# p-m-mueller/saddle_point_petsc

Measured on AMD Instinct MI355X. Metric: FGMRES iterations/sec + achieved HBM GB/s on A-block SpMV, 1/2/4/8 MI355X, higher is better.
Workload: dtype f64

## Files before the change

### include/spk.h

```cpp
#ifndef SPK_H
#define SPK_H

#include <stdint.h>

#ifdef __cplusplus
extern "C" {
#endif

#define SPK_VERSION 100

typedef struct spk_ctx spk_ctx;

enum { SPK_OK = 0, SPK_ERR_ARG = -1, SPK_ERR_HIP = -2, SPK_ERR_STATE = -3,
       SPK_ERR_COMM = -4, SPK_ERR_NOMEM = -5, SPK_ERR_UNSUPPORTED = -6 };

enum { SPK_MEM_HOST = 0, SPK_MEM_DEVICE = 1 };

enum { SPK_BLOCK_A00 = 0, SPK_BLOCK_A10 = 1 };

enum { SPK_PC_NONE = 0, SPK_PC_JACOBI = 1, SPK_PC_SCHUR = 2 };
enum { SPK_SCHUR_DIAG = 0, SPK_SCHUR_LOWER = 1, SPK_SCHUR_UPPER = 2, SPK_SCHUR_FULL = 3 };
enum { SPK_ORTHOG_CGS = 0, SPK_ORTHOG_MGS = 1 };
enum { SPK_REFINE_NEVER = 0, SPK_REFINE_IFNEEDED = 1, SPK_REFINE_ALWAYS = 2 };
enum { SPK_SPMV_CSR = 0 };
// ... 181 lines not shown
int spk_kernel_mdot(spk_ctx *ctx, int64_t n, int32_t nv, const double *V, int64_t ldv,
                    const double *w, double *h);
int spk_kernel_maxpy(spk_ctx *ctx, int64_t n, int32_t nv, const double *a, const double *V,
                     int64_t ldv, double *w, double *nrm2);
int spk_time_spmv(spk_ctx *ctx, int warmup, int reps, double *ms_per_launch);
int spk_time_kernel(spk_ctx *ctx, const char *which, int nv, int warmup, int reps,
                    double *ms_per_launch);

int spk_debug_finish_timeout(spk_ctx *ctx, int timeout_ms);

int spk_debug_wave_sums(spk_ctx *ctx, int na, const double *in, double *out);

#define SPK_DEBUG_MARKER (-7777777.0)
int spk_debug_vec_shape(spk_ctx *ctx, int64_t n, int32_t *out);
typedef struct spk_debug_mdot_opts {
    int64_t n, n_dot;
    int32_t nv, nv2;
    int32_t split, done;
    double pad;
} spk_debug_mdot_opts;
int spk_debug_mdot(spk_ctx *ctx, const spk_debug_mdot_opts *o, const double *V, const double *V2, const double *w, double *out);
typedef struct spk_debug_maxpy_opts {
    int64_t n, n_dot, n_bd;
    double sign, pad;
    int32_t nv, nv_live;
    int32_t want_norm;
    int32_t m, bd_mode;
    int32_t w1side, pyth, done;
} spk_debug_maxpy_opts;
int spk_debug_maxpy(spk_ctx *ctx, const spk_debug_maxpy_opts *o, const double *V, const double *a, double *w, const double *bd,
                    const double *dots, double *tb, double *red, double *w1side, double *nrm_out);
int spk_debug_cycle_norm(spk_ctx *ctx, int64_t n, int64_t n_dot, int64_t n_bd, int32_t m, double pad, double *x, const double *sa,
                         const double *sb, const double *bd, double *red, double *w1side);
int spk_debug_schur_w(spk_ctx *ctx, int64_t nl, int32_t m, int32_t fact, int32_t done, double pad, const double *W, const double *L,
                      const double *x, const double *src, const double *dinv, double *y);
int spk_debug_pack_bd(spk_ctx *ctx, int64_t n, int32_t m, const double *bd, double *bdp, int32_t *bad);
typedef struct spk_debug_head_opts {
    int64_t nl;
    int32_t m, packed, fact, jacobi, want_wl, reserved;
    double pad;
} spk_debug_head_opts;
int spk_debug_cycle_head(spk_ctx *ctx, const spk_debug_head_opts *o, double *v, const double *nrm, const double *w1raw,
                         const double *dinv, const double *bd, const double *shat, const double *gram, double *z, double *c,
                         double *wl);

int spk_debug_gs_stamps(spk_ctx *ctx, uint64_t *out);

int spk_debug_set_wait_bound(spk_ctx *ctx, uint32_t ticks);

int spk_debug_time_products(spk_ctx *ctx, int32_t max_launches);
int spk_get_product_timing(spk_ctx *ctx, int32_t *launches, double *mean_ms, double *median_ms, double *min_ms, double *max_ms,
                           int32_t *gated, double *gated_mean_ms);

int spk_partition_slab(int64_t nlines, int64_t line_rows, int rank, int nranks,
                       int64_t *row_begin, int64_t *row_end);
int spk_partition_split(int64_t row_begin, int32_t nrows_local, const int32_t *rowptr,
                        const int32_t *colidx, const double *val,
                        int32_t *d_rowptr, int32_t *d_colidx, double *d_val,
                        int32_t *o_rowptr, int32_t *o_colidx, double *o_val,
                        int32_t *garray, int64_t *nnz_d, int64_t *nnz_o, int32_t *n_ghost);

#ifdef __cplusplus
}
#endif
#endif
```

### saddle_point_petsc_amd/_lib.py

```python
import ctypes as C
import os

import numpy as np

_HERE = os.path.dirname(os.path.abspath(__file__))
LIB_PATH = os.path.join(_HERE, "libspk.so")

i32p = np.ctypeslib.ndpointer(np.int32, flags="C_CONTIGUOUS")
f64p = np.ctypeslib.ndpointer(np.float64, flags="C_CONTIGUOUS")


class SpkError(RuntimeError):
    def __init__(self, code, msg):
        super().__init__(f"libspk error {code}: {msg}")
        self.code = code


class Opts(C.Structure):
    _fields_ = [
        ("restart", C.c_int32), ("max_it", C.c_int32), ("rtol", C.c_double),
        ("abstol", C.c_double), ("dtol", C.c_double), ("guess_nonzero", C.c_int32),
        ("orthog", C.c_int32), ("check_every", C.c_int32), ("fused", C.c_int32),
        ("cgs_refine", C.c_int32), ("single_reduce", C.c_int32), ("iteration_form", C.c_int32), ("reserved", C.c_int32),
    ]
# ... 107 lines not shown
    _hip_preloaded = _preload_hip_runtime()
    L = C.CDLL(LIB_PATH)
    rts = hip_runtimes_mapped()
    if len(rts) > 1:
        raise ImportError("two HIP runtimes are mapped into this process (" + ", ".join(rts) + "): libspk.so would not find the "
                          "GPU.  Import saddle_point_petsc_amd before anything else that loads a HIP runtime of its own, or set "
                          "LD_LIBRARY_PATH so that both resolve libamdhip64.so.7 to the same file.")
    vp, i32, i64, dbl = C.c_void_p, C.c_int32, C.c_int64, C.c_double
    L.spk_version.restype = C.c_int
    L.spk_last_error.restype = C.c_char_p
    L.spk_last_error.argtypes = [vp]
    L.spk_default_opts.argtypes = [C.POINTER(Opts)]
    L.spk_default_opts.restype = None
    L.spk_create.argtypes = [C.POINTER(vp), C.c_int]
    L.spk_destroy.argtypes = [vp]
    L.spk_comm_unique_id.argtypes = [C.c_char_p]
    L.spk_comm_init_rccl.argtypes = [vp, C.c_int, C.c_int, C.c_char_p]
    L.spk_comm_init_host.argtypes = [vp, C.c_int, C.c_int, C.POINTER(HostComm)]
    L.spk_local_group_create.argtypes = [C.POINTER(vp), C.c_int]
    L.spk_local_group_destroy.argtypes = [vp]
    L.spk_comm_init_local.argtypes = [vp, vp, C.c_int]
    L.spk_comm_enable_peer.argtypes = [vp, C.POINTER(i32)]
    L.spk_comm_backend.restype = C.c_char_p
    L.spk_comm_backend.argtypes = [vp]
    L.spk_comm_get_info.argtypes = [vp, C.POINTER(CommInfo)]
    L.spk_debug_peer_allreduce_loopback.argtypes = [vp, C.c_int, C.c_int, C.c_int, f64p, f64p]
    L.spk_debug_finish_timeout.argtypes = [vp, C.c_int]
    L.spk_debug_set_wait_bound.argtypes = [vp, C.c_uint32]
    L.spk_debug_wave_sums.argtypes = [vp, C.c_int, f64p, f64p]
    L.spk_debug_vec_shape.argtypes = [vp, i64, i32p]
    L.spk_debug_mdot.argtypes = [vp, C.POINTER(DebugMdotOpts), vp, vp, f64p, f64p]
    L.spk_debug_maxpy.argtypes = [vp, C.POINTER(DebugMaxpyOpts), vp, f64p, f64p, vp, vp, vp, f64p, vp, vp]
    L.spk_debug_cycle_norm.argtypes = [vp, i64, i64, i64, i32, dbl, f64p, vp, vp, vp, f64p, vp]
    L.spk_debug_schur_w.argtypes = [vp, i64, i32, i32, i32, dbl, f64p, f64p, f64p, vp, vp, f64p]
    L.spk_debug_pack_bd.argtypes = [vp, i64, i32, f64p, vp, C.POINTER(i32)]
    L.spk_debug_cycle_head.argtypes = [vp, C.POINTER(DebugHeadOpts), f64p, f64p, vp, f64p, vp, vp, vp, f64p, vp, vp]
    L.spk_debug_gs_stamps.argtypes = [vp, np.ctypeslib.ndpointer(np.uint64, flags="C_CONTIGUOUS")]
    L.spk_debug_time_products.argtypes = [vp, C.c_int32]
    L.spk_get_product_timing.argtypes = [vp, C.POINTER(C.c_int32)] + [C.POINTER(C.c_double)] * 4 + [C.POINTER(C.c_int32), C.POINTER(C.c_double)]
    L.spk_set_block.argtypes = [vp, C.c_int, i64, i32, i64, i32p, i32p, f64p]
    L.spk_set_block_laplace.argtypes = [vp, C.c_int, C.c_int, vp, C.c_int, C.c_int, vp]
    L.spk_assemble_laplace_csr.argtypes = [vp, C.c_int, C.c_int, i64, i64, vp, C.c_int, C.c_int, i32p, i32p, f64p, vp]
    L.spk_set_block_laplace3d.argtypes = [vp, C.c_int, C.c_int, C.c_int, vp, C.c_int, C.c_int, vp]
    L.spk_assemble_laplace3d_csr.argtypes = [vp, C.c_int, C.c_int, C.c_int, i64, i64, vp, C.c_int, C.c_int, i32p, i32p, f64p, vp]
    L.spk_get_assembly_seconds.argtypes = [vp, C.POINTER(dbl)]
    L.spk_pc_setup.argtypes = [vp, C.c_int, C.c_int]
    L.spk_pc_set_inner.argtypes = [vp, C.c_int, C.c_double]
    L.spk_default_amg_opts.argtypes = [C.POINTER(AmgOpts)]
    L.spk_default_amg_opts.restype = None
    L.spk_pc_set_amg.argtypes = [vp, C.POINTER(AmgOpts)]
    L.spk_get_amg_info.argtypes = [vp, C.POINTER(AmgInfo)]
    L.spk_get_amg_level.argtypes = [vp, C.c_int, C.c_int, C.POINTER(i32), C.POINTER(i32), C.POINTER(i64), vp, vp, vp]
    L.spk_get_amg_aggregates.argtypes = [vp, C.c_int, C.POINTER(i32), vp]
    L.spk_amg_build_host.argtypes = [i32, i32p, i32p, f64p, C.POINTER(AmgOpts), C.POINTER(vp)]
    L.spk_amg_refresh_host.argtypes = [vp, vp]
    L.spk_amg_destroy_host.argtypes = [vp]
    L.spk_pc_set_amg_reuse.argtypes = [vp, C.c_int]
    L.spk_get_amg_reuse_info.argtypes = [vp, C.POINTER(i32), C.POINTER(dbl)]
    L.spk_amg_host_info.argtypes = [vp, C.POINTER(AmgInfo)]
    L.spk_amg_host_level.argtypes = [vp, C.c_int, C.c_int, C.POINTER(i32), C.POINTER(i32), C.POINTER(i64), vp, vp, vp]
    L.spk_amg_host_aggregates.argtypes = [vp, C.c_int, C.POINTER(i32), vp]
    L.spk_pc_set_schur_pre.argtypes = [vp, C.c_int]
    L.spk_get_schur_matrix.argtypes = [vp, f64p]
    L.spk_get_schur_setup_seconds.argtypes = [vp, C.POINTER(dbl)]
    L.spk_get_schur_diag.argtypes = [vp, f64p]
    L.spk_get_jacobi_diag.argtypes = [vp, f64p]
# ... 81 lines not shown
```

### saddle_point_petsc_amd/csrc/spk_api.cpp

```cpp
#include <algorithm>
#include <cmath>
#include <cstdlib>
#include <cstring>
#include <string>

#include "spk_internal.hpp"

namespace spk {
void rccl_unique_id(void *id128);
}

static thread_local std::string g_create_error;
namespace spk {
void set_create_error(const std::string &m) { g_create_error = m; }
}

#define SPK_TRY(ctx)                                                     \
    if (!(ctx)) return SPK_ERR_ARG;                                      \
    try {                                                                \
        if (hipSetDevice((ctx)->device) != hipSuccess)                   \
            spk::fail(SPK_ERR_HIP, "hipSetDevice(%d) failed", (ctx)->device);

#define SPK_CATCH(ctx)                                                   \
    }                                                                    \
// ... 670 lines not shown
    spk::DevBuf<double> dV, dw, da, dbd, ddots, dtb, dred, dside, dnrm;
    spk::DevBuf<int32_t> ddone, dnv;
    dbg_upload(dV, V, o->nv, n, ld, o->pad);
    dbg_upload(dw, w, 1, n, ld, o->pad);
    dbg_upload(dbd, bd, rows, n, ld, o->pad);
    da.upload(a, (size_t)o->nv, 8);
    dbg_fill(dred, (size_t)(1 + m), SPK_DEBUG_MARKER);
    dbg_fill(dside, (size_t)std::max(m, 1), SPK_DEBUG_MARKER);
    dbg_fill(dnrm, (size_t)(1 + m), SPK_DEBUG_MARKER);
    spk::k::PythArgs py{};
    py.m = -1;
    if (o->pyth) {
        ddots.upload(dots, (size_t)(live + m + 1), 8);
        dtb.upload(tb, (size_t)(o->nv + 1) * 8, 8);
        py = spk::k::PythArgs{m, ddots.p, dtb.p, dnrm.p};
    }
    if (o->nv_live >= 0) dnv.upload(&o->nv_live, 1, 3);
    const int32_t *done = dbg_done(ddone, o->done);
    spk::k::maxpy(dV.p, ld, o->nv, o->nv_live >= 0 ? dnv.p : nullptr, da.p, o->sign, dw.p, n, o->n_dot,
                  c->fin(o->want_norm ? dred.p : nullptr), done, c->stream, rows ? dbd.p : nullptr, ld, o->n_bd, m,
                  o->w1side ? dside.p : nullptr, o->pyth ? &py : nullptr, o->bd_mode == 2);
    SPK_HIP(hipStreamSynchronize(c->stream));
    c->check_device_error();
    SPK_HIP(hipMemcpy(w, dw.p, sizeof(double) * (size_t)n, hipMemcpyDeviceToHost));
    SPK_HIP(hipMemcpy(red, dred.p, sizeof(double) * (size_t)(1 + m), hipMemcpyDeviceToHost));
    if (w1side && m) SPK_HIP(hipMemcpy(w1side, dside.p, sizeof(double) * (size_t)m, hipMemcpyDeviceToHost));
    if (o->pyth) {
        SPK_HIP(hipMemcpy(nrm_out, dnrm.p, sizeof(double) * (size_t)(1 + m), hipMemcpyDeviceToHost));
        SPK_HIP(hipMemcpy(tb, dtb.p, sizeof(double) * (size_t)(o->nv + 1) * 8, hipMemcpyDeviceToHost));
    }
    SPK_CATCH(c)
}

int spk_debug_cycle_norm(spk_ctx *c, int64_t n, int64_t n_dot, int64_t n_bd, int32_t m, double pad, double *x, const double *sa,
                         const double *sb, const double *bd, double *red, double *w1side)
{
    SPK_TRY(c)
    if (!x || !red || n <= 0 || n_dot < 0 || n_dot > n || n_bd < 0 || n_bd + m > n || m < 0 || m > 8 || (m && (!bd || !w1side)) ||
        (!sa != !sb))
        spk::fail(SPK_ERR_ARG, "spk_debug_cycle_norm: bad arguments");
    c->ensure_scratch();
    const int64_t ld = dbg_ld(n);
    spk::DevBuf<double> dx, dsa, dsb, dbd, dred, dside;
    dbg_upload(dx, sa ? nullptr : x, 1, n, ld, pad);
    if (sa) {
        dbg_upload(dsa, sa, 1, n, ld, pad);
        dbg_upload(dsb, sb, 1, n, ld, pad);
    }
    dbg_upload(dbd, bd, m, n, ld, pad);
    dbg_fill(dred, (size_t)(1 + m), SPK_DEBUG_MARKER);
    dbg_fill(dside, (size_t)std::max<int>(m, 1), SPK_DEBUG_MARKER);
    spk::k::sqnorm_bd(dx.p, n, n_dot, dbd.p, ld, n_bd, m, dside.p, c->fin(dred.p), nullptr, c->stream, sa ? dsa.p : nullptr,
                      sa ? dsb.p : nullptr);
    SPK_HIP(hipStreamSynchronize(c->stream));
    c->check_device_error();
    SPK_HIP(hipMemcpy(x, dx.p, sizeof(double) * (size_t)n, hipMemcpyDeviceToHost));
    SPK_HIP(hipMemcpy(red, dred.p, sizeof(double) * (size_t)(1 + m), hipMemcpyDeviceToHost));
    if (m) SPK_HIP(hipMemcpy(w1side, dside.p, sizeof(double) * (size_t)m, hipMemcpyDeviceToHost));
    SPK_CATCH(c)
}

int spk_debug_schur_w(spk_ctx *c, int64_t nl, int32_t m, int32_t fact, int32_t done, double pad, const double *W, const double *L,
                      const double *x, const double *src, const double *dinv, double *y)
{
    SPK_TRY(c)
    if (!W || !L || !x || !y || nl <= 0 || m < 1 || m > 8 || fact < SPK_SCHUR_DIAG || fact > SPK_SCHUR_FULL || (src && dinv))
        spk::fail(SPK_ERR_ARG, "spk_debug_schur_w: bad arguments");
    c->ensure_scratch();
    const int64_t ld = dbg_ld(nl + m);
    spk::DevBuf<double> dW, dL, dx, dsrc, ddinv, dy;
    spk::DevBuf<int32_t> ddone;
    dbg_upload(dW, W, m, nl, ld, 0.0);
    dL.upload(L, (size_t)m * m, 8);
    dbg_upload(dx, x, 1, nl + m, ld, pad);
    if (src) dbg_upload(dsrc, src, 1, nl, ld, pad);
    if (dinv) dbg_upload(ddinv, dinv, 1, nl, ld, pad);
    dbg_upload(dy, nullptr, 1, nl + m, ld, SPK_DEBUG_MARKER);
    const int32_t *gate = dbg_done(ddone, done);
    const spk::k::SchurW w{dW.p, ld, m, dL.p};
    if (fact == SPK_SCHUR_DIAG || fact == SPK_SCHUR_UPPER) spk::k::schur_w_y1(w, fact, dx.p + nl, dy.p + nl, gate, c->stream);
    else spk::k::schur_w_dot(w, dx.p, nl, dx.p + nl, dy.p + nl, c->fin(nullptr), gate, c->stream);
    if (fact == SPK_SCHUR_UPPER || fact == SPK_SCHUR_FULL)
        spk::k::schur_w_out(w, src ? dsrc.p : dx.p, dinv ? ddinv.p : nullptr, dy.p + nl, dy.p, nl, gate, c->stream);
    SPK_HIP(hipStreamSynchronize(c->stream));
    c->check_device_error();
    SPK_HIP(hipMemcpy(y, dy.p, sizeof(double) * (size_t)ld, hipMemcpyDeviceToHost));
// ... 313 lines not shown
```

### saddle_point_petsc_amd/csrc/spk_device.hpp

```cpp
#pragma once
#include "spk_internal.hpp"
#include "spk_gs_stamps.hpp"

#include <cmath>
#include <cstdlib>
#include <type_traits>

namespace spk {
namespace k {

constexpr int kThreads = 256;
constexpr int kWave = 64;
constexpr int kVT = 1024;
constexpr int kVWaves = kVT / kWave;
constexpr int kVecUnroll = 4;
constexpr int kVecMaxBlocks = 256;

__device__ __forceinline__ double wave_sum(double v)
{
#pragma unroll
    for (int off = kWave / 2; off > 0; off >>= 1) v += __shfl_down(v, off, kWave);
    return v;
}

// ... 495 lines not shown
{
    const GivensPre pre = givens_prefetch(gr.ka, gr.loc, gr.h);
    if (gr.fin_n > 0) {
        double *red = lds;
        double *slot = gr.fin_partials + (size_t)gr.fin_n * kPartialLd;
        double lam2 = 0.0;
        if (threadIdx.x == 0) lam2 = peek(slot);
        final_reduce<2>(gr.fin_partials, gr.fin_n, kPartialLd, 1, red, gr.fe);
        if (threadIdx.x == 0) {
            publish(slot, __longlong_as_double((long long)kSentinelBits));
            red[0] = red[0] + lam2;
        }
        __syncthreads();
        if (gr.ar.P) peer_allreduce_block(gr.ar, red, 1, gr.nrm2);
        else if (threadIdx.x == 0) gr.nrm2[0] = red[0];
        __syncthreads();
    }
    if (gr.sc && threadIdx.x == 0) gr.sc[gr.loc + 1] = inv_norm(*gr.nrm2);
    givens_block_lds<true>(gr.ka, gr.loc, gr.h, gr.nrm2, lds + kThreads, kMaxNv + 2, &pre);
}

void givens_rider_alone(const GivensRider &gr, const int32_t *done, hipStream_t s);
inline GivensRider no_rider()
{
    GivensRider g{};
    g.loc = -1;
    return g;
}

struct RowTail {
    const int32_t *bt_rowptr, *bt_colidx;
    const double *bt_val, *lam;
    OffDiag od;
};

template <bool RIDE>
__device__ __forceinline__ int product_prologue(const int32_t *done, const GivensRider &gr, double *lds)
{
    if (done && *done) return -1;
    if (RIDE && blockIdx.x == 0) {
        givens_rider(gr, lds);
        return -1;
    }
    return (int)blockIdx.x - (RIDE ? 1 : 0);
}
__device__ __forceinline__ int xcd_tile(int bx, int tiles_per_xcd) { return (bx & 7) * tiles_per_xcd + (bx >> 3); }

__device__ __forceinline__ void row_tail_bt(const RowTail &t, int k, int k1, double &s)
{
    for (; k < k1; ++k) s = __builtin_fma(t.bt_val[k], t.lam[t.bt_colidx[k]], s);
}
__device__ __forceinline__ void row_tail_add(const RowTail &t, int64_t row, double &s, bool bt)
{
    if (t.od.rowptr)
        for (int k = t.od.rowptr[row]; k < t.od.rowptr[row + 1]; ++k) s = __builtin_fma(t.od.val[k], t.od.xg[t.od.colidx[k]], s);
    if (bt) row_tail_bt(t, t.bt_rowptr[row], t.bt_rowptr[row + 1], s);
}
constexpr int kBtPre = 4;
struct BtPre {
    int k0, k1;
    double v[kBtPre], l[kBtPre];
    __device__ __forceinline__ void load(const RowTail &t, int64_t row)
    {
        k0 = t.bt_rowptr[row];
        k1 = t.bt_rowptr[row + 1];
#pragma unroll
// ... 7 lines not shown
    {
#pragma unroll
        for (int j = 0; j < kBtPre; ++j)
            if (k0 + j < k1) s = __builtin_fma(v[j], l[j], s);
        row_tail_bt(t, k0 + kBtPre, k1, s);
    }
};

__device__ __forceinline__ float sweep_update(float y, float omega, float d, float x, float s)
{
#pragma clang fp contract(off)
    return y + ((omega * d) * (x - s));
}

struct ProductLaunch {
    RowTail tail;
    GivensRider gr;
    const int32_t *done;
    int nride;
    bool acc, ride, bt;
    size_t rider_lds;
};
inline bool product_is_empty(int64_t nrows, const GivensRider *rider, const int32_t *done, hipStream_t s)
{
    if (nrows == 0 && rider) givens_rider_alone(*rider, done, s);
    return nrows == 0;
}
inline ProductLaunch make_product_launch(const CsrDev *bt, const double *lam, const OffDiag *od, const GivensRider *rider,
                                         const int32_t *done, bool accumulate)
{
    if (bt && rider) fail(SPK_ERR_ARG, "A-block product: B^T rows and a rider in one launch");
    ProductLaunch p{};
    p.tail = RowTail{bt ? bt->rowptr.p : nullptr, bt ? bt->colidx.p : nullptr, bt ? bt->val.p : nullptr, lam,
                     od ? *od : OffDiag{nullptr, nullptr, nullptr, nullptr}};
    p.gr = rider ? *rider : no_rider();
    p.done = done;
    p.nride = rider ? 1 : 0;
    p.acc = accumulate;
    p.ride = rider != nullptr;
    p.bt = bt != nullptr;
    p.rider_lds = rider ? sizeof(double) * (size_t)(kThreads + 4 * (kMaxNv + 2) + 4) : 0;
    return p;
}
template <class F>
inline void dispatch_product(bool acc, bool ride, bool bt, F &&f)
{
    using Y = std::true_type;
    using N = std::false_type;
    if (bt) acc ? f(Y{}, N{}, Y{}) : f(N{}, N{}, Y{});
    else if (acc) ride ? f(Y{}, Y{}, N{}) : f(Y{}, N{}, N{});
    else ride ? f(N{}, Y{}, N{}) : f(N{}, N{}, N{});
}

struct WsShape {
    int U, grid;
    bool on;
};
inline WsShape ws_shape(int64_t n2)
{
    WsShape v;
    static const int knob = [] { const char *e = getenv("SPK_VEC_WS"); return e ? atoi(e) : -1; }();
    v.on = n2 < (int64_t)kVecMaxBlocks * 2048 && knob != 0;
    v.U = n2 >= (int64_t)kVecMaxBlocks * 64 * 8 ? 8 : (n2 >= (int64_t)kVecMaxBlocks * 64 * 4 ? 4 : 2);
    if (knob == 2 || knob == 4 || knob == 8) v.U = knob;
    int64_t tiles = (n2 + 64 * v.U - 1) / (64 * v.U);
    if (tiles < 1) tiles = 1;
    v.grid = (int)(tiles < kVecMaxBlocks ? tiles : kVecMaxBlocks);
// ... 200 lines not shown
```

### saddle_point_petsc_amd/csrc/spk_internal.hpp

```cpp
#pragma once
#include <hip/hip_runtime.h>

#include <algorithm>
#include <chrono>
#include <cstdint>
#include <cstdio>
#include <functional>
#include <memory>
#include <string>
#include <vector>

#include <hip/hip_ext.h>

#include "spk_host.hpp"
#include "spk_amg.hpp"

namespace spk {

#define SPK_HIP(call)                                                                  \
    do {                                                                               \
        hipError_t e_ = (call);                                                        \
        if (e_ != hipSuccess)                                                          \
            ::spk::fail(SPK_ERR_HIP, "%s failed: %s (%s:%d)", #call, hipGetErrorString(e_), \
                        __FILE__, __LINE__);                                           \
// ... 227 lines not shown

struct SolverWork {
    DevBuf<double> vec;
    DevBuf<double> out, hist;
    DevBuf<unsigned char> state;
    void *pin = nullptr;
    hipEvent_t ev[2] = {nullptr, nullptr};
    void ensure(int64_t ld, int nvec, int32_t hist_cap, size_t state_bytes);
    ~SolverWork();
};

namespace k {
constexpr int kMaxNv = 64;
constexpr int kBigNv = 1024;
constexpr int kPartialLd = 64;
constexpr int kMaxBlocks = 2048;
constexpr int kBTile = 512;

void build_tiles(const int32_t *rowptr, int32_t nrows, std::vector<int32_t> &tile_row);
void arm_partials(double *p, size_t n, hipStream_t s);
struct Finish;
void finish_probe(const Finish &f, hipStream_t s);
void wave_sums_probe(int na, const double *in, double *out, hipStream_t s);
void vec_shapes_probe(int64_t n, int32_t *out);

struct Finish {
    double *partials;
    double *out;
    PeerAR ar;
    int32_t *err = nullptr;
    uint32_t fin_ticks = 400000000u;
};

struct OffDiag {
    const int32_t *rowptr, *colidx;
    const double *val, *xg;
};
struct SendRanges {
    int n;
    int32_t r0[4], len[4], off[4];
    double *buf;
    int peer;
    uint32_t seq, timeout_ms;
    unsigned long long *remote[4];
    const unsigned long long *mine;
    int32_t nrecv;
    double *xghost;
    int32_t *err;
    unsigned long long *stats;
};

struct GivensRider;
void spmv(const CsrDev &A, const double *x, double *y, const CsrDev *bt, const double *lam,
          const int32_t *done, hipStream_t s, bool accumulate = false, const OffDiag *od = nullptr,
          const GivensRider *rider = nullptr);
void spmv_bcsr(const BcsrDev &A, const double *x, double *y, const CsrDev *bt, const double *lam,
               const int32_t *done, hipStream_t s, bool accumulate = false, const OffDiag *od = nullptr,
               const GivensRider *rider = nullptr);
void build_btiles(const int32_t *browptr, int32_t nbrows, std::vector<int32_t> &tile_brow);
constexpr int kB3Tile = 256;
void spmv_bcsr3(const Bcsr3Dev &A, const double *x, double *y, const CsrDev *bt, const double *lam,
                const int32_t *done, hipStream_t s, bool accumulate = false, const OffDiag *od = nullptr,
                const GivensRider *rider = nullptr);
void build_b3tiles(const int32_t *browptr, int32_t nbrows, std::vector<int32_t> &tile_brow);
constexpr int kDictMaxPat = 1024, kDictMaxBlk = 1024, kDictSlots = 8192, kDictLdsMax = 48 * 1024;
void spmv_dict(const DictDev &A, const double *x, double *y, const CsrDev *bt, const double *lam, const int32_t *done,
// ... 41 lines not shown
               double *vbot, int32_t *fail, hipStream_t s);
void assemble_laplace(int mx, int my, int j0, int j1, const double *kappa, int apply_bc, int32_t *rowptr, int32_t *colidx, double *val,
                      double *f, hipStream_t s);
int64_t assemble_laplace_grid(int mx, int j0, int j1);
void assemble_laplace3d(int mx, int my, int mz, int k0, int k1, const double *kappa, int apply_bc, int32_t *rowptr, int32_t *colidx,
                        double *val, double *f, hipStream_t s);
int64_t assemble_laplace3d_grid(int mx, int my, int k0, int k1);
void kappa_check(const double *kappa, int64_t ne, int32_t *flag, hipStream_t s);
void wide_dot(const WideDev &B, const double *x, const Finish &f, const int32_t *done, hipStream_t s,
              const int32_t *rowmap = nullptr);
void schur_diag_rows(const CsrDev &B, const double *dinv, double *shat, hipStream_t s);
void wide_dot_jacobi(const WideDev &B, const double *x, const double *dinv, const Finish &f,
                     const int32_t *done, hipStream_t s);
void scatter_row(const int32_t *colidx, const double *val, int k0, int k1, const double *dinv,
                 double *dense, hipStream_t s);
void sum_slots(const double *slots, int nslots, int ld, int count, double *out, hipStream_t s);
void mdot(const double *V, int64_t ldv, int nv, const double *w, int64_t n, int64_t n_dot,
          const Finish &f, const int32_t *done, hipStream_t s, const double *V2 = nullptr, int nv2 = 0,
          int v2_split = 0);
struct PythArgs {
    int m;
    const double *dots;
    double *tb;
    double *nrm_out;
};
void maxpy(const double *V, int64_t ldv, int nv, const int32_t *nv_dev, const double *a,
           double coef_sign, double *w, int64_t n, int64_t n_dot, const Finish &f,
           const int32_t *done, hipStream_t s, const double *bd = nullptr, int64_t ldb = 0, int64_t n_bd = 0, int m = 0,
           double *w1side = nullptr, const PythArgs *pyth = nullptr, int bd_packed = 0);
void build_bd(const CsrDev &Bt, const double *dinv, int m, int64_t ldb, double *bd, hipStream_t s);
void pack_bd(const double *bd, int64_t ldb, int64_t n, int m, double *bdp, int32_t *bad, hipStream_t s);
void sqnorm_bd(double *x, int64_t n, int64_t n_dot, const double *bd, int64_t ldb, int64_t n_bd, int m,
               double *w1side, const Finish &f, const int32_t *done, hipStream_t s, const double *sa = nullptr,
               const double *sb = nullptr);
void scale_dev(double *x, int64_t n, const double *alpha_dev, const int32_t *done, hipStream_t s);
void axpby(double a, const double *x, double b, double *y, int64_t n, const int32_t *done, hipStream_t s);
void sqnorm(const double *x, int64_t n_dot, const Finish &f, const int32_t *done, hipStream_t s);
void sqnorm_sub(const double *sa, const double *sb, double *x, int64_t n, int64_t n_dot, const Finish &f, const int32_t *done,
                hipStream_t s);
void gather(const double *x, const int32_t *idx, int64_t n, double *out, const int32_t *done, hipStream_t s);
void peer_allreduce(const PeerAR &a, double *buf, int count, hipStream_t s);
void peer_allreduce_loopback(const PeerAR &a, double *buf, int count, hipStream_t s);
void peer_exchange(const PeerHalo &h, const double *sendbuf, double *recvbuf, hipStream_t s);
void peer_exchange_bulk(const PeerBulk &h, const double *sendbuf, double *recvbuf, hipStream_t s);
void jacobi(const double *dinv, const double *x, double *y, int64_t n, const int32_t *done, hipStream_t s);
void extract_diag_inv(const CsrDev &A, double *dinv, hipStream_t s);
void bt_update(int mode, const CsrDev &Bt, const double *dinv, const double *x0, const double *y1,
               double *y0, const int32_t *done, hipStream_t s, double *scratch = nullptr);
void cvt_scale_f32(const double *x, const float *d32, float omega, float *x32, float *y32, int64_t n,
                   const int32_t *done, hipStream_t s);
void jacobi_sweep_f32(const CsrDev &A, const float *val32, const float *d32, float omega, const float *x32,
                      const float *yin, float *yout, const int32_t *done, hipStream_t s);
void sweep_offdiag_f32(const CsrDev &Ao, const int32_t *rows, const float *d32, float omega, const double *xg,
                       float *y, const int32_t *done, hipStream_t s);
void gather_f32(const float *x, const int32_t *idx, int64_t n, double *out, const int32_t *done, hipStream_t s);
void cvt_f32_out(const float *y32, double *y, int mode, int64_t n, const int32_t *done, hipStream_t s);
void cvt_vals_f32(const double *v, float *v32, int64_t n, hipStream_t s);
void schur_y1(int fact, int m, const double *x1, const double *t, const double *shat, double *y1,
              const int32_t *done, hipStream_t s);
void copy_small(const double *src, double *dst, int n, const int32_t *done, hipStream_t s);
struct SchurW {
    const double *W;
    int64_t ldw;
    int m;
    const double *L;
};
void schur_w_dot(const SchurW &w, const double *x0, int64_t nl, const double *x1, double *y1, const Finish &f,
// ... 421 lines not shown
```

### saddle_point_petsc_amd/csrc/spk_k_dict.hip

```cpp
#include "spk_dict.hpp"

#include <climits>

namespace spk {
namespace k {

template <int BS, bool ACC, bool RIDE, bool BT, int U3>
__global__ __launch_bounds__(kThreads) void spmv_dict_kernel(DictArgs d, const double *__restrict__ x, double *__restrict__ y,
                                                             RowTail tail, const int32_t *__restrict__ done, GivensRider gr)
{
#pragma clang fp contract(off)
    extern __shared__ __attribute__((aligned(16))) char smem[];
    const int bx = product_prologue<RIDE>(done, gr, reinterpret_cast<double *>(smem));
    int c0, c1;
    if (bx < 0 || !dict_chunk_range(d, bx, c0, c1)) return;
    int br = c0 * kDictChunk + (int)threadIdx.x;
    int tidn = br < d.nbrows ? (int)d.tid[br] : -1;
    dict_load_lds(d, (d.nclass + 1) * BS * BS, smem);
    const DictTables T = dict_tables(d, smem);

    for (int ch = c0; ch < c1; ++ch) {
        const int tc = tidn;
        const int brc = br;
        br += kDictChunk;
// ... 147 lines not shown
    __builtin_amdgcn_sched_barrier(0);
    Dict2Stage<KM, ACC> SA, SB;
    dict2_issue_stream<KM, ACC>(d, yr, dict_rowof(d, c0, c1), SA);
    if (Dict2TableWords<KM, UNI>::fits(d)) {
        tw.commit(d, T, 16);
    } else {
        dict_load_lds(d, (d.nclass + 1) * 4, smem);
        dict_prepare_types<KM>(d, T, 16);
    }
    dict2_issue_gather<KM, ACC>(xr, T.tent, tA, dict_rowof(d, c0, c1), SA);
    tA = (int)d.tid[dict_rowof(d, c0 + 2, c1)];

    auto compute = [&](int ch, const Dict2Stage<KM, ACC> &S) {
        const int brc = ch * kDictChunk + (int)threadIdx.x;
        double s[2] = {0.0, 0.0};
#pragma unroll
        for (int g = 0; g < KM; ++g) {
            const double2 *cb = T.cv + (size_t)S.cls[g] * 4;
            if (UNI) {
                const int lo = (int)(uint32_t)S.w[g], hi = (int)(uint32_t)(S.w[g] >> 32);
                s[0] += dict_decode(__builtin_amdgcn_sbfe(lo, 0u, (unsigned)d.uw[0]), cb[0]) * S.xv[g].x;
                s[0] += dict_decode(lo >> (32 - d.uw[1]), cb[1]) * S.xv[g].y;
                s[1] += dict_decode(__builtin_amdgcn_sbfe(hi, 0u, (unsigned)d.uw[2]), cb[2]) * S.xv[g].x;
                s[1] += dict_decode(hi >> (32 - d.uw[3]), cb[3]) * S.xv[g].y;
            } else {
                const int32_t *fb = T.fl + (size_t)S.cls[g] * 4;
                s[0] += dict_decode(dict_field2(S.w[g], fb[0]), cb[0]) * S.xv[g].x;
                s[0] += dict_decode(dict_field2(S.w[g], fb[1]), cb[1]) * S.xv[g].y;
                s[1] += dict_decode(dict_field2(S.w[g], fb[2]), cb[2]) * S.xv[g].x;
                s[1] += dict_decode(dict_field2(S.w[g], fb[3]), cb[3]) * S.xv[g].y;
            }
        }
        if (has_tail && brc < d.nbrows) {
#pragma unroll
            for (int r = 0; r < 2; ++r) row_tail_add(tail, 2 * (int64_t)brc + r, s[r], BT);
        }
        if (ACC) {
            s[0] += S.yv.x;
            s[1] += S.yv.y;
        }
        double2 o;
        o.x = s[0];
        o.y = s[1];
        __builtin_amdgcn_raw_buffer_store_b128(__builtin_bit_cast(b128_t, o), yr, (int)((uint32_t)brc * 16u), 0, 0);
    };
    auto issue = [&](int ch, int &t, Dict2Stage<KM, ACC> &S) {
        dict2_issue_stream<KM, ACC>(d, yr, dict_rowof(d, ch, c1), S);
        dict2_issue_gather<KM, ACC>(xr, T.tent, t, dict_rowof(d, ch, c1), S);
        t = (int)d.tid[dict_rowof(d, ch + 2, c1)];
        __builtin_amdgcn_sched_barrier(0);
    };
    for (int ch = c0;; ch += 2) {
        issue(ch + 1, tB, SB);
        compute(ch, SA);
        if (ch + 1 >= c1) break;
        issue(ch + 2, tA, SA);
        compute(ch + 1, SB);
        if (ch + 2 >= c1) break;
    }
}

void spmv_dict(const DictDev &A, const double *x, double *y, const CsrDev *bt, const double *lam, const int32_t *done,
               hipStream_t s, bool accumulate, const OffDiag *odp, const GivensRider *rider)
{
    if (product_is_empty(A.nbrows, rider, done, s)) return;
    if (spmv_dict3(A, x, y, bt, lam, done, s, accumulate, odp, rider)) return;
    const ProductLaunch p = make_product_launch(bt, lam, odp, rider, done, accumulate);
    int grid = 0;
// ... 390 lines not shown
```

### saddle_point_petsc_amd/csrc/spk_k_vec.hip

```cpp
#include "spk_device.hpp"

namespace spk {
namespace k {

__global__ void arm_partials_kernel(double *p, size_t n)
{
    const size_t i = (size_t)blockIdx.x * blockDim.x + threadIdx.x;
    if (i < n) p[i] = __longlong_as_double((long long)kSentinelBits);
}
void arm_partials(double *p, size_t n, hipStream_t s)
{
    hipLaunchKernelGGL(arm_partials_kernel, dim3((unsigned)((n + 255) / 256)), dim3(256), 0, s, p, n);
}

__global__ __launch_bounds__(256) void finish_probe_kernel(double *partials, double *out, FinErr fe)
{
    __shared__ double scratch[256];
    if (blockIdx.x + 1 < gridDim.x) {
        if (threadIdx.x == 0) publish(partials + (size_t)blockIdx.x * kPartialLd, 1.0);
        return;
    }
    __syncthreads();
    final_reduce(partials, gridDim.x, kPartialLd, 1, scratch, fe);
    if (threadIdx.x == 0) out[0] = scratch[0];
// ... 837 lines not shown
    for (int r = 0; r < m; ++r) bd[(size_t)r * ldb + i] = 0.0;
    for (int k = rowptr[i]; k < rowptr[i + 1]; ++k) bd[(size_t)colidx[k] * ldb + i] += val[k] * dinv[i];
}
void build_bd(const CsrDev &Bt, const double *dinv, int m, int64_t ldb, double *bd, hipStream_t s)
{
    if (Bt.nrows == 0) return;
    hipLaunchKernelGGL(build_bd_kernel, dim3((Bt.nrows + kThreads - 1) / kThreads), dim3(kThreads), 0, s,
                       Bt.rowptr.p, Bt.colidx.p, Bt.val.p, Bt.nrows, dinv, m, ldb, bd);
}

__global__ __launch_bounds__(kThreads) void pack_bd_kernel(const double *__restrict__ bd, int64_t ldb, int64_t n, int m,
                                                           double *__restrict__ bdp, int32_t *__restrict__ bad)
{
    const int64_t i = (int64_t)blockIdx.x * kThreads + threadIdx.x;
    if (i >= n) return;
    for (int q = 0; 2 * q + 1 < m; ++q) {
        const double a = bd[(size_t)(2 * q) * ldb + i], b = bd[(size_t)(2 * q + 1) * ldb + i];
        if ((i & 1) ? a != 0.0 : b != 0.0) *bad = 1;
        bdp[(size_t)q * ldb + i] = (i & 1) ? b : a;
    }
}
void pack_bd(const double *bd, int64_t ldb, int64_t n, int m, double *bdp, int32_t *bad, hipStream_t s)
{
    if (n == 0) return;
    hipLaunchKernelGGL(pack_bd_kernel, dim3((unsigned)((n + kThreads - 1) / kThreads)), dim3(kThreads), 0, s, bd, ldb, n, m, bdp, bad);
}

template <int MP>
__global__ __launch_bounds__(512) void sqnorm_bd_kernel(double *__restrict__ x, int64_t n2, int64_t n_dot,
                                                        const double *__restrict__ bd, int64_t ldb, int64_t n_bd,
                                                        int m, double *__restrict__ w1side,
                                                        double *__restrict__ partials, double *__restrict__ out,
                                                        FinErr fe, const int32_t *__restrict__ done,
                                                        const double *__restrict__ sa, const double *__restrict__ sb)
{
    if (done && *done) return;
    constexpr int T = 512, NR = MP + 1, W = T / kWave;
    __shared__ double red[(W * NR > T) ? W * NR : T];
    double acc[NR];
#pragma unroll
    for (int r = 0; r < NR; ++r) acc[r] = 0.0;
    for (int64_t i = (int64_t)blockIdx.x * T + threadIdx.x; i < n2; i += (int64_t)gridDim.x * T) {
        double2 v;
        if (sa) {
            const double2 av = reinterpret_cast<const double2 *>(sa)[i], bv = reinterpret_cast<const double2 *>(sb)[i];
            v.x = av.x - bv.x;
            v.y = av.y - bv.y;
            reinterpret_cast<double2 *>(x)[i] = v;
        } else {
            v = reinterpret_cast<const double2 *>(x)[i];
        }
        if (2 * i < n_dot) acc[0] += v.x * v.x;
        if (2 * i + 1 < n_dot) acc[0] += v.y * v.y;
        {
            const int64_t e0 = 2 * i - n_bd;
            if (e0 >= 0 && e0 < m) w1side[e0] = v.x;
            if (e0 + 1 >= 0 && e0 + 1 < m) w1side[e0 + 1] = v.y;
        }
#pragma unroll
        for (int r = 0; r < MP; ++r) {
            if (r < m) {
                const double2 e = reinterpret_cast<const double2 *>(bd + (size_t)r * ldb)[i];
                if (2 * i < n_bd) acc[1 + r] += e.x * v.x;
                if (2 * i + 1 < n_bd) acc[1 + r] += e.y * v.y;
            }
        }
    }
    const int lane = threadIdx.x & 63, wave = threadIdx.x >> 6;
#pragma unroll
    for (int r = 0; r < NR; ++r) {
        const double s = wave_sum(acc[r]);
        if (lane == 0) red[wave * NR + r] = s;
    }
    __syncthreads();
    if ((int)threadIdx.x < NR) {
        double t = 0.0;
#pragma unroll
        for (int j = 0; j < W; ++j) t += red[j * NR + threadIdx.x];
        if ((int)threadIdx.x <= m) publish(partials + (size_t)blockIdx.x * kPartialLd + threadIdx.x, t);
    }
    if (!arrive_last(gridDim.x)) return;
    final_reduce(partials, gridDim.x, kPartialLd, 1 + m, red, fe);
    if ((int)threadIdx.x < 1 + m) out[threadIdx.x] = red[threadIdx.x];
}
void sqnorm_bd(double *x, int64_t n, int64_t n_dot, const double *bd, int64_t ldb, int64_t n_bd, int m,
               double *w1side, const Finish &f, const int32_t *done, hipStream_t s, const double *sa, const double *sb)
{
    const int64_t n2 = (n + 1) / 2;
    const int grid = vec_grid(n2, 512);
    if (m <= 4)
        hipLaunchKernelGGL(sqnorm_bd_kernel<4>, dim3(grid), dim3(512), 0, s, x, n2, n_dot, bd, ldb, n_bd, m, w1side, f.partials, f.out, FinErr{f.err, f.fin_ticks}, done, sa, sb);
    else
        hipLaunchKernelGGL(sqnorm_bd_kernel<8>, dim3(grid), dim3(512), 0, s, x, n2, n_dot, bd, ldb, n_bd, m, w1side, f.partials, f.out, FinErr{f.err, f.fin_ticks}, done, sa, sb);
}

__global__ void sum_slots_kernel(const double *__restrict__ slots, int nslots, int ld, int count,
                                 double *__restrict__ out)
{
    const int i = blockIdx.x * blockDim.x + threadIdx.x;
    if (i >= count) return;
    double s = 0.0;
    for (int r = 0; r < nslots; ++r) s += slots[(size_t)r * ld + i];
    out[i] = s;
}
void sum_slots(const double *slots, int nslots, int ld, int count, double *out, hipStream_t s)
{
    if (count == 0) return;
    hipLaunchKernelGGL(sum_slots_kernel, dim3((count + 63) / 64), dim3(64), 0, s, slots, nslots, ld, count, out);
}


}
}
```

### saddle_point_petsc_amd/csrc/spk_solver.cpp

```cpp
#include <algorithm>
#include <chrono>
#include <cstddef>
#include <cstdlib>
#include <cstring>
#include <numeric>

#include "spk_internal.hpp"

using namespace spk;

void spk_ctx::ensure_scratch()
{
    if (!partials.p) {
        partials.alloc((size_t)k::kMaxBlocks * k::kPartialLd);
        k::arm_partials(partials.p, partials.n, stream);
        SPK_HIP(hipStreamSynchronize(stream));
    }
    if (!errw.p) errw.alloc(4);
    if (!small.p) small.alloc(512);
    if (!y1tmp.p) y1tmp.alloc(64);
    if (!ttmp.p) ttmp.alloc(64);
}

void spk_ctx::check_device_error()
// ... 685 lines not shown
            if (loc >= its_cap) break;
            const int32_t *done = &c->kst.p->skip_iter;
            double *w = r.Vj(loc + 1);
            double *db = p.big ? c->bigdots.p : r.dotsbuf(loc), *nb = r.nrmbuf(loc);
            if (un3) {
                if (un3_iteration(r, cs, loc, done)) break;
            } else {
                if (p.product == FgmresPlan::kStep) {
                    op_pc_apply(c, r.Vj(loc), r.Zj(loc), done);
                    op_mult(c, r.Zj(loc), w, done, false, true);
                } else {
                    head_product(r, cs, loc, w, done);
                }
                if (p.orth == FgmresPlan::kOrthMgs) orth_mgs(r, loc, w, db, nb, done);
                else if (p.orth == FgmresPlan::kOrthSingle) orth_single(r, cs, loc, w, db, nb, done);
                else orth_cgs(r, loc, w, db, nb, done);
                if (!p.head || p.big) {
                    k::krylov_givens(c->ka, loc, db, nb, s);
                    if (!p.head) k::scale_dev(w, N, inv_tt, done, s);
                }
            }
            if (o.check_every > 0 && (loc + 1) % o.check_every == 0 && loc + 1 < mk) {
                SPK_HIP(hipMemcpyAsync(&st, c->kst.p, sizeof st, hipMemcpyDeviceToHost, s));
                SPK_HIP(hipStreamSynchronize(s));
                cs.stop = st.done != 0 || st.skip_iter != 0;
            }
        }
        if (finished || (pend_check && read_state())) break;
        if (p.head && cs.last >= 0) cs.pend_h = r.dotsbuf(cs.last), cs.pend_n = r.nrmbuf(cs.last), cs.pend_loc = cs.last;
        const k::GivensRider pend{c->ka, cs.pend_loc, cs.pend_h, cs.pend_n, nullptr, nullptr, 0, k::FinErr{nullptr, 0}, k::PeerAR{}};
        k::krylov_cycle_end(c->ka, s, un3 ? c->basis_sc.p : nullptr, mk, cs.pend_loc >= 0 ? &pend : nullptr);
        k::maxpy(r.Z, ld, mk, &c->kst.p->loc_done, c->ka.nrs, 1.0, x, N, 0, c->fin(nullptr), nullptr, s);
        op_mult(c, x, c->tmp.p, done);
        if (p.schur) k::sqnorm_bd(r.Vj(0), N, n_dot, c->bd.p, ld, r.nl, r.m, r.w1side, c->fin(r.nrmbuf(1)), done, s, b, c->tmp.p);
        else k::sqnorm_sub(b, c->tmp.p, r.Vj(0), N, n_dot, c->fin(r.nrmbuf(1)), done, s);
        ++cycles;
        SPK_HIP(hipGetLastError());
    }
    finish_solve(c, st, cycles, t0, c->ka.hist, c->ka.hist_cap, res, history, history_cap);
}

}
```

### saddle_point_petsc_amd/solver.py

```python
import ctypes as C
import math

import numpy as np

from ._lib import lib, Opts, Result, MatCSR, SpkError, AmgOpts, AmgInfo

PC_NONE, PC_JACOBI, PC_SCHUR = 0, 1, 2
SCHUR_DIAG, SCHUR_LOWER, SCHUR_UPPER, SCHUR_FULL = 0, 1, 2, 3
BLOCK_A00, BLOCK_A10 = 0, 1
MEM_HOST, MEM_DEVICE = 0, 1
NORM_UNPRECONDITIONED, NORM_NATURAL = 0, 1
DIVERGED_INDEFINITE_PC = -8
DIVERGED_INDEFINITE_MAT = -10
PIPECGRR_TAU_DEFAULT = 1e-6
_NORMS = {"unpreconditioned": NORM_UNPRECONDITIONED, "natural": NORM_NATURAL}
SCHUR_PRE_SELFP_DIAG, SCHUR_PRE_FULL = 0, 1
_SCHUR_PRES = {"selfp": SCHUR_PRE_SELFP_DIAG, "full": SCHUR_PRE_FULL}


def default_opts(**kw):
    o = Opts()
    lib.spk_default_opts(C.byref(o))
    for k, v in kw.items():
        if not hasattr(o, k):
# ... 269 lines not shown
        V = self._f64(V, (np.shape(V)[0], n))
        nv = V.shape[0]
        a = self._f64(a, (nv,))
        mode = 0 if bd is None else (2 if packed else 1)
        bd = None if bd is None else self._f64(bd, ((m // 2 if packed else m), n))
        live = nv if nv_live < 0 else nv_live
        dots = tb = None
        if pyth is not None:
            dots = self._f64(pyth["dots"], (live + m + 1,))
            tb = self._f64(pyth["tb"], (nv + 1, 8)).copy()
        o = DebugMaxpyOpts(n, n if n_dot is None else n_dot, n_bd, float(sign), float(pad), nv, nv_live, int(want_norm), m, mode,
                           int(w1side), int(pyth is not None), int(done))
        red, side, nrm_out = np.zeros(1 + m), np.zeros(max(m, 1)), np.zeros(1 + m)
        self._chk(lib.spk_debug_maxpy(self.h, C.byref(o), self._ptr(V), a, w, self._ptr(bd), self._ptr(dots), self._ptr(tb), red,
                                      self._ptr(side), self._ptr(nrm_out)))
        return dict(w=w, red=red, w1side=side[:m], nrm_out=nrm_out, tb=tb)

    def debug_cycle_norm(self, x, bd, n_bd, n_dot=None, sub=None, pad=0.0):
        bd = self._f64(bd)
        m = bd.shape[0]
        sa = sb = None
        if sub is not None:
            sa, sb = self._f64(sub[0]), self._f64(sub[1])
            x = np.zeros_like(sa)
        x = self._f64(x).copy()
        n = x.shape[0]
        if m and bd.shape != (m, n):
            raise ValueError("debug_cycle_norm: bd must be (m, n)")
        red, side = np.zeros(1 + m), np.zeros(max(m, 1))
        self._chk(lib.spk_debug_cycle_norm(self.h, n, n if n_dot is None else n_dot, n_bd, m, float(pad), x, self._ptr(sa),
                                           self._ptr(sb), self._ptr(bd) if m else None, red, self._ptr(side)))
        return dict(x=x, red=red, w1side=side[:m])

    def debug_schur_w(self, W, L, x, fact=SCHUR_FULL, src=None, dinv=None, done=-1, pad=0.0):
        W = self._f64(W)
        m, nl = W.shape
        L = self._f64(L, (m, m))
        x = self._f64(x, (nl + m,))
        src = None if src is None else self._f64(src, (nl,))
        dinv = None if dinv is None else self._f64(dinv, (nl,))
        y = np.zeros((nl + m + 255) // 256 * 256)
        self._chk(lib.spk_debug_schur_w(self.h, nl, m, int(fact), int(done), float(pad), W, L, x, self._ptr(src), self._ptr(dinv), y))
        return y

    def debug_pack_bd(self, bd):
        bd = self._f64(bd)
        m, n = bd.shape
        bdp = np.zeros((max(m // 2, 1), n))
        bad = C.c_int32(-1)
        self._chk(lib.spk_debug_pack_bd(self.h, n, m, bd, self._ptr(bdp), C.byref(bad)))
        return bdp[:m // 2], bad.value

    def debug_cycle_head(self, v, nrm, dinv, w1raw=None, bd=None, shat=None, gram=None, fact=SCHUR_FULL, packed=0, jacobi=False,
                         want_wl=False, pad=0.0):
        from ._lib import DebugHeadOpts
        dinv = self._f64(dinv)
        nl = dinv.shape[0]
        nrm = self._f64(nrm)
        m = nrm.shape[0] - 1
        v = self._f64(v, (nl + m,)).copy()
        if m:
            w1raw, shat, gram = self._f64(w1raw, (m,)), self._f64(shat, (m,)), self._f64(gram, (m, m))
            bd = self._f64(bd, ((m // 2 if packed else m), nl))
        else:
            w1raw = shat = gram = bd = None
        z = np.zeros(nl + m)
# ... 469 lines not shown
```

Before: 7006.

## Use packed B-border planes in cycle-end norm and batch B^T tail loads

The Schur-path residual norm at cycle end now reads the packed border matrix, which has half as many planes with two rows interleaved, instead of m full planes. This cuts the bytes streamed per restart cycle. The dictionary SpMV tail also prefetches the B^T row data for both rows before accumulating, rather than walking each row serially. Both paths are on by default and can be switched off with SPK_TAIL_BATCH=0. The batched prefetch may raise register pressure in the SpMV kernel.

```diff
diff --git a/include/spk.h b/include/spk.h
--- a/include/spk.h
+++ b/include/spk.h
@@ -237,6 +237,8 @@
                     const double *dots, double *tb, double *red, double *w1side, double *nrm_out);
 int spk_debug_cycle_norm(spk_ctx *ctx, int64_t n, int64_t n_dot, int64_t n_bd, int32_t m, double pad, double *x, const double *sa,
                          const double *sb, const double *bd, double *red, double *w1side);
+int spk_debug_cycle_norm_packed(spk_ctx *ctx, int64_t n, int64_t n_dot, int64_t n_bd, int32_t m, double pad, double *x,
+                                const double *sa, const double *sb, const double *bdp, double *red, double *w1side);
 int spk_debug_schur_w(spk_ctx *ctx, int64_t nl, int32_t m, int32_t fact, int32_t done, double pad, const double *W, const double *L,
                       const double *x, const double *src, const double *dinv, double *y);
 int spk_debug_pack_bd(spk_ctx *ctx, int64_t n, int32_t m, const double *bd, double *bdp, int32_t *bad);
diff --git a/saddle_point_petsc_amd/_lib.py b/saddle_point_petsc_amd/_lib.py
--- a/saddle_point_petsc_amd/_lib.py
+++ b/saddle_point_petsc_amd/_lib.py
@@ -163,6 +163,7 @@
     L.spk_debug_mdot.argtypes = [vp, C.POINTER(DebugMdotOpts), vp, vp, f64p, f64p]
     L.spk_debug_maxpy.argtypes = [vp, C.POINTER(DebugMaxpyOpts), vp, f64p, f64p, vp, vp, vp, f64p, vp, vp]
     L.spk_debug_cycle_norm.argtypes = [vp, i64, i64, i64, i32, dbl, f64p, vp, vp, vp, f64p, vp]
+    L.spk_debug_cycle_norm_packed.argtypes = [vp, i64, i64, i64, i32, dbl, f64p, vp, vp, vp, f64p, vp]
     L.spk_debug_schur_w.argtypes = [vp, i64, i32, i32, i32, dbl, f64p, f64p, f64p, vp, vp, f64p]
     L.spk_debug_pack_bd.argtypes = [vp, i64, i32, f64p, vp, C.POINTER(i32)]
     L.spk_debug_cycle_head.argtypes = [vp, C.POINTER(DebugHeadOpts), f64p, f64p, vp, f64p, vp, vp, vp, f64p, vp, vp]
diff --git a/saddle_point_petsc_amd/csrc/spk_api.cpp b/saddle_point_petsc_amd/csrc/spk_api.cpp
--- a/saddle_point_petsc_amd/csrc/spk_api.cpp
+++ b/saddle_point_petsc_amd/csrc/spk_api.cpp
@@ -726,12 +726,24 @@
     SPK_CATCH(c)
 }
 
+static int debug_cycle_norm(spk_ctx *c, int64_t n, int64_t n_dot, int64_t n_bd, int32_t m, double pad, double *x, const double *sa,
+                            const double *sb, const double *bd, double *red, double *w1side, int packed);
 int spk_debug_cycle_norm(spk_ctx *c, int64_t n, int64_t n_dot, int64_t n_bd, int32_t m, double pad, double *x, const double *sa,
                          const double *sb, const double *bd, double *red, double *w1side)
 {
+    return debug_cycle_norm(c, n, n_dot, n_bd, m, pad, x, sa, sb, bd, red, w1side, 0);
+}
+int spk_debug_cycle_norm_packed(spk_ctx *c, int64_t n, int64_t n_dot, int64_t n_bd, int32_t m, double pad, double *x,
+                                const double *sa, const double *sb, const double *bdp, double *red, double *w1side)
+{
+    return debug_cycle_norm(c, n, n_dot, n_bd, m, pad, x, sa, sb, bdp, red, w1side, 1);
+}
+static int debug_cycle_norm(spk_ctx *c, int64_t n, int64_t n_dot, int64_t n_bd, int32_t m, double pad, double *x, const double *sa,
+                            const double *sb, const double *bd, double *red, double *w1side, int packed)
+{
     SPK_TRY(c)
     if (!x || !red || n <= 0 || n_dot < 0 || n_dot > n || n_bd < 0 || n_bd + m > n || m < 0 || m > 8 || (m && (!bd || !w1side)) ||
-        (!sa != !sb))
+        (!sa != !sb) || (packed && m % 2))
         spk::fail(SPK_ERR_ARG, "spk_debug_cycle_norm: bad arguments");
     c->ensure_scratch();
     const int64_t ld = dbg_ld(n);
@@ -741,11 +753,11 @@
         dbg_upload(dsa, sa, 1, n, ld, pad);
         dbg_upload(dsb, sb, 1, n, ld, pad);
     }
-    dbg_upload(dbd, bd, m, n, ld, pad);
+    dbg_upload(dbd, bd, packed ? m / 2 : m, n, ld, pad);
     dbg_fill(dred, (size_t)(1 + m), SPK_DEBUG_MARKER);
     dbg_fill(dside, (size_t)std::max<int>(m, 1), SPK_DEBUG_MARKER);
     spk::k::sqnorm_bd(dx.p, n, n_dot, dbd.p, ld, n_bd, m, dside.p, c->fin(dred.p), nullptr, c->stream, sa ? dsa.p : nullptr,
-                      sa ? dsb.p : nullptr);
+                      sa ? dsb.p : nullptr, packed);
     SPK_HIP(hipStreamSynchronize(c->stream));
     c->check_device_error();
     SPK_HIP(hipMemcpy(x, dx.p, sizeof(double) * (size_t)n, hipMemcpyDeviceToHost));
diff --git a/saddle_point_petsc_amd/csrc/spk_device.hpp b/saddle_point_petsc_amd/csrc/spk_device.hpp
--- a/saddle_point_petsc_amd/csrc/spk_device.hpp
+++ b/saddle_point_petsc_amd/csrc/spk_device.hpp
@@ -551,6 +551,7 @@
     const int32_t *bt_rowptr, *bt_colidx;
     const double *bt_val, *lam;
     OffDiag od;
+    int bt_serial = 0;
 };
 
 template <bool RIDE>
@@ -624,7 +625,7 @@
     if (bt && rider) fail(SPK_ERR_ARG, "A-block product: B^T rows and a rider in one launch");
     ProductLaunch p{};
     p.tail = RowTail{bt ? bt->rowptr.p : nullptr, bt ? bt->colidx.p : nullptr, bt ? bt->val.p : nullptr, lam,
-                     od ? *od : OffDiag{nullptr, nullptr, nullptr, nullptr}};
+                     od ? *od : OffDiag{nullptr, nullptr, nullptr, nullptr}, tail_batch_on() ? 0 : 1};
     p.gr = rider ? *rider : no_rider();
     p.done = done;
     p.nride = rider ? 1 : 0;
diff --git a/saddle_point_petsc_amd/csrc/spk_internal.hpp b/saddle_point_petsc_amd/csrc/spk_internal.hpp
--- a/saddle_point_petsc_amd/csrc/spk_internal.hpp
+++ b/saddle_point_petsc_amd/csrc/spk_internal.hpp
@@ -283,6 +283,11 @@
     uint32_t fin_ticks = 400000000u;
 };
 
+inline bool tail_batch_on()
+{
+    const char *e = getenv("SPK_TAIL_BATCH");
+    return !(e && e[0] == '0' && !e[1]);
+}
 struct OffDiag {
     const int32_t *rowptr, *colidx;
     const double *val, *xg;
@@ -390,7 +395,7 @@
 void pack_bd(const double *bd, int64_t ldb, int64_t n, int m, double *bdp, int32_t *bad, hipStream_t s);
 void sqnorm_bd(double *x, int64_t n, int64_t n_dot, const double *bd, int64_t ldb, int64_t n_bd, int m,
                double *w1side, const Finish &f, const int32_t *done, hipStream_t s, const double *sa = nullptr,
-               const double *sb = nullptr);
+               const double *sb = nullptr, int bd_packed = 0);
 void scale_dev(double *x, int64_t n, const double *alpha_dev, const int32_t *done, hipStream_t s);
 void axpby(double a, const double *x, double b, double *y, int64_t n, const int32_t *done, hipStream_t s);
 void sqnorm(const double *x, int64_t n_dot, const Finish &f, const int32_t *done, hipStream_t s);
diff --git a/saddle_point_petsc_amd/csrc/spk_k_dict.hip b/saddle_point_petsc_amd/csrc/spk_k_dict.hip
--- a/saddle_point_petsc_amd/csrc/spk_k_dict.hip
+++ b/saddle_point_petsc_amd/csrc/spk_k_dict.hip
@@ -203,8 +203,20 @@
             }
         }
         if (has_tail && brc < d.nbrows) {
-#pragma unroll
-            for (int r = 0; r < 2; ++r) row_tail_add(tail, 2 * (int64_t)brc + r, s[r], BT);
+            if (BT && tail.bt_serial) {
+#pragma unroll
+                for (int r = 0; r < 2; ++r) row_tail_add(tail, 2 * (int64_t)brc + r, s[r], true);
+            } else {
+#pragma unroll
+                for (int r = 0; r < 2; ++r) row_tail_add(tail, 2 * (int64_t)brc + r, s[r], false);
+                if (BT) {
+                    BtPre pre[2];
+#pragma unroll
+                    for (int r = 0; r < 2; ++r) pre[r].load(tail, 2 * (int64_t)brc + r);
+#pragma unroll
+                    for (int r = 0; r < 2; ++r) pre[r].add(tail, s[r]);
+                }
+            }
         }
         if (ACC) {
             s[0] += S.yv.x;
diff --git a/saddle_point_petsc_amd/csrc/spk_k_vec.hip b/saddle_point_petsc_amd/csrc/spk_k_vec.hip
--- a/saddle_point_petsc_amd/csrc/spk_k_vec.hip
+++ b/saddle_point_petsc_amd/csrc/spk_k_vec.hip
@@ -893,7 +893,7 @@
                                                         int m, double *__restrict__ w1side,
                                                         double *__restrict__ partials, double *__restrict__ out,
                                                         FinErr fe, const int32_t *__restrict__ done,
-                                                        const double *__restrict__ sa, const double *__restrict__ sb)
+                                                        const double *__restrict__ sa, const double *__restrict__ sb, int packed)
 {
     if (done && *done) return;
     constexpr int T = 512, NR = MP + 1, W = T / kWave;
@@ -918,12 +918,23 @@
             if (e0 >= 0 && e0 < m) w1side[e0] = v.x;
             if (e0 + 1 >= 0 && e0 + 1 < m) w1side[e0 + 1] = v.y;
         }
-#pragma unroll
-        for (int r = 0; r < MP; ++r) {
-            if (r < m) {
-                const double2 e = reinterpret_cast<const double2 *>(bd + (size_t)r * ldb)[i];
-                if (2 * i < n_bd) acc[1 + r] += e.x * v.x;
-                if (2 * i + 1 < n_bd) acc[1 + r] += e.y * v.y;
+        if (packed) {
+#pragma unroll
+            for (int q = 0; q < MP / 2; ++q) {
+                if (2 * q < m) {
+                    const double2 e = reinterpret_cast<const double2 *>(bd + (size_t)q * ldb)[i];
+                    if (2 * i < n_bd) acc[1 + 2 * q] += e.x * v.x;
+                    if (2 * i + 1 < n_bd) acc[2 + 2 * q] += e.y * v.y;
+                }
+            }
+        } else {
+#pragma unroll
+            for (int r = 0; r < MP; ++r) {
+                if (r < m) {
+                    const double2 e = reinterpret_cast<const double2 *>(bd + (size_t)r * ldb)[i];
+                    if (2 * i < n_bd) acc[1 + r] += e.x * v.x;
+                    if (2 * i + 1 < n_bd) acc[1 + r] += e.y * v.y;
+                }
             }
         }
     }
@@ -945,14 +956,16 @@
     if ((int)threadIdx.x < 1 + m) out[threadIdx.x] = red[threadIdx.x];
 }
 void sqnorm_bd(double *x, int64_t n, int64_t n_dot, const double *bd, int64_t ldb, int64_t n_bd, int m,
-               double *w1side, const Finish &f, const int32_t *done, hipStream_t s, const double *sa, const double *sb)
-{
+               double *w1side, const Finish &f, const int32_t *done, hipStream_t s, const double *sa, const double *sb,
+               int bd_packed)
+{
+    if (bd_packed && m % 2) fail(SPK_ERR_ARG, "sqnorm_bd: packed planes hold an even number of rows");
     const int64_t n2 = (n + 1) / 2;
     const int grid = vec_grid(n2, 512);
     if (m <= 4)
-        hipLaunchKernelGGL(sqnorm_bd_kernel<4>, dim3(grid), dim3(512), 0, s, x, n2, n_dot, bd, ldb, n_bd, m, w1side, f.partials, f.out, FinErr{f.err, f.fin_ticks}, done, sa, sb);
+        hipLaunchKernelGGL(sqnorm_bd_kernel<4>, dim3(grid), dim3(512), 0, s, x, n2, n_dot, bd, ldb, n_bd, m, w1side, f.partials, f.out, FinErr{f.err, f.fin_ticks}, done, sa, sb, bd_packed);
     else
-        hipLaunchKernelGGL(sqnorm_bd_kernel<8>, dim3(grid), dim3(512), 0, s, x, n2, n_dot, bd, ldb, n_bd, m, w1side, f.partials, f.out, FinErr{f.err, f.fin_ticks}, done, sa, sb);
+        hipLaunchKernelGGL(sqnorm_bd_kernel<8>, dim3(grid), dim3(512), 0, s, x, n2, n_dot, bd, ldb, n_bd, m, w1side, f.partials, f.out, FinErr{f.err, f.fin_ticks}, done, sa, sb, bd_packed);
 }
 
 __global__ void sum_slots_kernel(const double *__restrict__ slots, int nslots, int ld, int count,
diff --git a/saddle_point_petsc_amd/csrc/spk_solver.cpp b/saddle_point_petsc_amd/csrc/spk_solver.cpp
--- a/saddle_point_petsc_amd/csrc/spk_solver.cpp
+++ b/saddle_point_petsc_amd/csrc/spk_solver.cpp
@@ -741,7 +741,10 @@
         k::krylov_cycle_end(c->ka, s, un3 ? c->basis_sc.p : nullptr, mk, cs.pend_loc >= 0 ? &pend : nullptr);
         k::maxpy(r.Z, ld, mk, &c->kst.p->loc_done, c->ka.nrs, 1.0, x, N, 0, c->fin(nullptr), nullptr, s);
         op_mult(c, x, c->tmp.p, done);
-        if (p.schur) k::sqnorm_bd(r.Vj(0), N, n_dot, c->bd.p, ld, r.nl, r.m, r.w1side, c->fin(r.nrmbuf(1)), done, s, b, c->tmp.p);
+        if (p.schur) {
+            const bool pk = p.bpk && k::tail_batch_on();
+            k::sqnorm_bd(r.Vj(0), N, n_dot, pk ? c->bdpk.p : c->bd.p, ld, r.nl, r.m, r.w1side, c->fin(r.nrmbuf(1)), done, s, b, c->tmp.p, pk);
+        }
         else k::sqnorm_sub(b, c->tmp.p, r.Vj(0), N, n_dot, c->fin(r.nrmbuf(1)), done, s);
         ++cycles;
         SPK_HIP(hipGetLastError());
diff --git a/saddle_point_petsc_amd/solver.py b/saddle_point_petsc_amd/solver.py
--- a/saddle_point_petsc_amd/solver.py
+++ b/saddle_point_petsc_amd/solver.py
@@ -325,6 +325,22 @@
                                            self._ptr(sb), self._ptr(bd) if m else None, red, self._ptr(side)))
         return dict(x=x, red=red, w1side=side[:m])
 
+    def debug_cycle_norm_packed(self, x, bdp, n_bd, n_dot=None, sub=None, pad=0.0):
+        bdp = self._f64(bdp)
+        m = 2 * bdp.shape[0]
+        sa = sb = None
+        if sub is not None:
+            sa, sb = self._f64(sub[0]), self._f64(sub[1])
+            x = np.zeros_like(sa)
+        x = self._f64(x).copy()
+        n = x.shape[0]
+        if m == 0 or bdp.shape != (m // 2, n):
+            raise ValueError("debug_cycle_norm_packed: bdp must be (m / 2, n), m > 0")
+        red, side = np.zeros(1 + m), np.zeros(m)
+        self._chk(lib.spk_debug_cycle_norm_packed(self.h, n, n if n_dot is None else n_dot, n_bd, m, float(pad), x, self._ptr(sa),
+                                                  self._ptr(sb), self._ptr(bdp), red, self._ptr(side)))
+        return dict(x=x, red=red, w1side=side)
+
     def debug_schur_w(self, W, L, x, fact=SCHUR_FULL, src=None, dinv=None, done=-1, pad=0.0):
         W = self._f64(W)
         m, nl = W.shape
```

After: 6998, median of 3. No clear change (-0.1%).
